# annikabrundyn/driving-dirty

Measured on AMD Instinct MI355X. Metric: 6-view scenes/sec fwd+bwd, roadmap model bs=32, higher is better.
Workload: dtype f32

## Files before the change

driving-dirty_amd/_lib.py:

```python
import ctypes as C
import os

import torch

from .build import LIB

if os.environ.get("DD_HOTPATH_LIB"):
    LIB = os.environ["DD_HOTPATH_LIB"]

_i32, _i64, _f32, _p = C.c_int32, C.c_int64, C.c_float, C.c_void_p


class ConvDesc(C.Structure):
    _fields_ = [(n, _i32) for n in ("batch", "height", "width", "cin_real", "cin_store", "cout",
                                    "ksize", "stride", "pad", "rows_per_task")]


class GConvDesc(C.Structure):
    _fields_ = [(n, _i32) for n in ("batch", "in_h", "in_w", "in_cstore", "in_coff", "cin", "out_h", "out_w",
                                    "omem_h", "omem_w", "out_cstore", "out_coff", "cout", "kh", "kw", "stride_h",
                                    "stride_w", "dil_h", "dil_w", "pad_h", "pad_w", "div_h", "div_w", "ostride_h",
                                    "ostride_w", "ooff_h", "ooff_w", "mask_pass_lo", "mask_pass_hi")]


class AdamTensor(C.Structure):
    _fields_ = [("p", _p), ("g", _p), ("m", _p), ("v", _p), ("n", _i64)]


_DP = C.POINTER(ConvDesc)
_GP = C.POINTER(GConvDesc)

SIGNATURES = {
    "dd_abi_version": (_i32, []),
    "dd_last_error": (C.c_char_p, []),
    "dd_clock_probe": (_i32, [_p, _i32, _i32, _p]),
    "dd_set_cu_budget": (_i32, [_i32]),
    "dd_set_adam_blocks_per_cu": (_i32, [_i32]),
    "dd_set_adam_spare_cus": (_i32, [_i32]),
    "dd_get_cu_budget": (_i32, []),
    "dd_stitch6": (_i32, [_p, _p, _p, _p, _i32, _i32, _i32, _i32, _p]),
    "dd_stitch6_ptrs": (_i32, [_p, _p, _i32, _i32, _i32, _p]),
    "dd_boxes_to_binary_map": (_i32, [_p, _i32, _p, _p, _i32, _p]),
    "dd_stitch6_u8": (_i32, [_p, _p, _i32, _i32, _i32, _p]),
    "dd_stitch6_u8_ptrs": (_i32, [_p, _p, _p, _i32, _i32, _i32, _i32, _p]),
    "dd_nchw_to_nhwc": (_i32, [_p, _p, _i32, _i32, _i32, _i32, _i32, _p]),
    "dd_subsample_nhwc4": (_i32, [_p, _p, _i32, _i32, _i32, _i32, _i32, _i32, _i32, _p]),
    "dd_subsample_nhwc4_u8_ptrs": (_i32, [_p, _p, _i32, _i32, _i32, _i32, _i32, _i32, _i32, _p]),
    "dd_copy_channels": (_i32, [_p, _p, _i64, _i32, _i32, _i32, _i32, _i32, _p]),
    "dd_copy_channels_window": (_i32, [_p, _p] + [_i32] * 16 + [_p]),
    "dd_deconv2x2_c32_fwd": (_i32, [_p, _p, _p, _p, _i32, _i32, _i32, _i32, _p]),
    "dd_deconv2x2_c32_fwd_slice": (_i32, [_p, _p, _p, _p, _i32, _i32, _i32, _i32, _i32, _i32, _p]),
    "dd_deconv2x2_c32_wgrad_workspace_bytes": (_i64, []),
    "dd_deconv2x2_c32_wgrad": (_i32, [_p, _p, _p, _p, _i32, _i32, _i32, _i32, _i32, _p, _i64, _p]),
    "dd_ssconv_dgrad_supported": (_i32, [_i32, _i32, _i32]),
    "dd_ssconv_dgrad": (_i32, [_p, _p, _p, _i32, _i32, _i32, _i32, _p]),
    "dd_ssconv_fwd": (_i32, [_p, _p, _p, _p, _i32, _i32, _i32, _i32, _i32, _p]),
    "dd_conv1x1_c32_c3_nchw": (_i32, [_p, _p, _p, _p, _i32, _i32, _i32, _p]),
    "dd_conv1ch_fwd": (_i32, [_p, _p, _p, _p, _i32, _i32, _i32, _i32, _p]),
    "dd_conv1ch_wgrad_workspace_bytes": (_i64, []),
    "dd_conv1ch_fwd_phase3": (_i32, [_p, _p, _p, _p, _p, _i32, _i32, _i32, _i32, _p]),
    "dd_conv1ch_wgrad_phase3": (_i32, [_p, _p, _p, _p, _i32, _i32, _i32, _p, _p]),
    "dd_phase3_scatter": (_i32, [_p, _p] + [_i32] * 8 + [_p]),
    "dd_phase3_gather": (_i32, [_p, _p] + [_i32] * 8 + [_p]),
    "dd_conv1ch_wgrad": (_i32, [_p, _p, _p, _p, _i32, _i32, _i32, _p, _p]),
    "dd_nhwc_to_nchw": (_i32, [_p, _p, _i32, _i32, _i32, _i32, _i32, _p]),
    "dd_conv_packed_floats": (_i64, [_DP, _i32]),
    "dd_conv_pack": (_i32, [_p, _p, _DP, _i32, _p]),
    "dd_conv_fwd": (_i32, [_p, _p, _p, _p, _p, _DP, _i32, _p]),
    "dd_conv_fwd_relu_bits": (_i32, [_p, _p, _p, _p, _p, _DP, _p]),
    "dd_conv_dgrad_relu_bits": (_i32, [_p, _p, _p, _p, _DP, _p]),
    "dd_conv_stats_floats": (_i64, []),
    "dd_conv_fwd_stats": (_i32, [_p, _p, _p, _p, _p, _p, _DP, _p]),
    "dd_bn2d_finalize": (_i32, [_p, _i64, _p, _p, _p, _p, _f32, _f32, _i32, _p, _p, _p, _p]),
    "dd_bn2d_stats": (_i32, [_p, _p, _i64, _p]),
    "dd_bn2d_apply_relu": (_i32, [_p, _p, _p, _i64, _p]),
    "dd_bn2d_workspace_bytes": (_i64, []),
    "dd_bn2d_bwd": (_i32, [_p, _p, _p, _p, _p, _p, _p, _p, _i64, _i32, _p, _p]),
    "dd_conv_dgrad_bn": (_i32, [_p, _p, _p, _p, _p, _DP, _p]),
    "dd_conv_wgrad_bn": (_i32, [_p, _p, _p, _p, _p, _p, _i64, _DP, _p]),
    "dd_pool4_bn_fwd": (_i32, [_p, _p, _p, _i32, _i32, _i32, _p]),
    "dd_pool4_bn_bwd": (_i32, [_p, _p, _p, _p, _i32, _i32, _i32, _p]),
    "dd_conv_dgrad": (_i32, [_p, _p, _p, _p, _DP, _p]),
    "dd_conv_wgrad_workspace_bytes": (_i64, [_DP]),
    "dd_conv_wgrad": (_i32, [_p, _p, _p, _p, _p, _i64, _DP, _p]),
    "dd_relu_bwd": (_i32, [_p, _p, _p, _i64, _p]),
    "dd_relu_sign_bits": (_i32, [_p, _p, _i64, _p]),
    "dd_relu_bwd_pad_bits": (_i32, [_p, _p, _p, _i32, _i32, _i32, _i32, _i32, _p]),
    "dd_pool4_fwd": (_i32, [_p, _p, _i32, _i32, _i32, _i32, _p]),
    "dd_pool4_relu_bwd": (_i32, [_p, _p, _p, _i32, _i32, _i32, _i32, _p]),
    "dd_pool4_relu_bwd_add": (_i32, [_p, _p, _p, _p, _i32, _i32, _i32, _i32, _p]),
    "dd_pool4_idx_elems": (_i64, [_i32, _i32, _i32, _i32]),
    "dd_pool4_fwd_idx": (_i32, [_p, _p, _p, _i32, _i32, _i32, _i32, _p]),
    "dd_pool4_idx_relu_bwd": (_i32, [_p, _p, _p, _i32, _i32, _i32, _i32, _p]),
    "dd_mlp_tail_supported": (_i32, [_i32] * 4),
    "dd_mlp_tail_fwd": (_i32, [_p] * 25 + [_i32] * 4 + [_f32] * 6 + [_i32, _p]),
    "dd_mlp_tail_bwd": (_i32, [_p] * 28 + [_i32] * 4 + [_f32] * 4 + [_i32, _p]),
    "dd_bn_relu_drop_fwd": (_i32, [_p] * 9 + [_i32, _i32, _f32, _f32, _f32, _i32, _p, _p]),
    "dd_bn_relu_drop_bwd": (_i32, [_p] * 12 + [_i32, _i32, _f32, _f32, _i32, _p]),
    "dd_loss_workspace_bytes": (_i64, [_i64]),
    "dd_bce_logits": (_i32, [_p, _p, _p, _p, _p, _i64, _f32, _p, _p]),
    "dd_bce_logits_u8": (_i32, [_p, _p, _p, _p, _p, _i64, _f32, _p, _p]),
    "dd_bce_logits_u8_ptrs": (_i32, [_p, _p, _i32, _i64, _p, _p, _p, _f32, _p, _p]),
    "dd_scale_by_device_scalar": (_i32, [_p, _p, _i64, _p]),
    "dd_sigmoid": (_i32, [_p, _p, _i64, _p]),
    "dd_sigmoid_bwd": (_i32, [_p, _p, _p, _i64, _p]),
    "dd_mse": (_i32, [_p, _p, _p, _p, _i64, _f32, _p, _p]),
    "dd_gconv_packed_floats": (_i64, [_GP]),
    "dd_gconv_pack": (_i32, [_p, _p, _GP, _i64, _i64, _i64, _i32, _i32, _i32, _p]),
    "dd_gconv_fwd": (_i32, [_p, _p, _p, _p, _p, _GP, _i32, _p]),
    "dd_gconv_wgrad_workspace_bytes": (_i64, [_GP]),
    "dd_gconv_wgrad": (_i32, [_p, _p, _p, _p, _GP, _i64, _i64, _i64, _i32, _i32, _i32, _i32, _p, _i64, _p]),
    "dd_dconv_supported": (_i32, [_GP]),
    "dd_dconv_packed_floats": (_i64, [_GP]),
    "dd_dconv_pack": (_i32, [_p, _p, _GP, _i64, _i64, _i64, _i32, _i32, _i32, _p]),
    "dd_dconv_fwd": (_i32, [_p, _p, _p, _p, _p, _GP, _i32, _p]),
    "dd_dconv_colsum_supported": (_i32, [_p, _i32, _i32]),
    "dd_dconv_colsum_workspace_bytes": (_i64, []),
    "dd_dconv_fwd_colsum": (_i32, [_p, _p, _p, _p, _p, _p, _i32, _p, _i64, _p]),
    "dd_dconv_split_supported": (_i32, [_GP]),
    "dd_dconv_split_input_bytes": (_i64, [_GP]),
    "dd_dconv_split_packed_bytes": (_i64, [_GP]),
    "dd_dconv_split_input": (_i32, [_p, _p, _GP, _p]),
    "dd_dconv_split_pack": (_i32, [_p, _p, _GP, _i64, _i64, _i64, _i32, _i32, _i32, _p]),
# ... 114 lines not shown
```

driving-dirty_amd/csrc/conv3x3.hip:

```cpp
#include <stdlib.h>

#include "dd_common.h"

namespace {

constexpr int EPI_BIAS_RELU_BITS = 5;
constexpr int EPI_RELU_BITS = 6;
constexpr int EPI_BIAS_STATS = 7;
constexpr int EPI_RELU_MASK_AFF = 8;
constexpr int EPI_RELU_BITS_W1 = 9;


template <int CIN, int S>
struct StripCfg {
  static constexpr int PXB = CIN * 4;
  static constexpr int CHUNKS = CIN / 4;
  static constexpr int NPX = 32 * S + 2;
  static constexpr int SLOTB = NPX * PXB;
  static constexpr int NCH = NPX * CHUNKS;
  static constexpr int NLOAD = (NCH + 63) / 64;
  static constexpr int SPILLB = (NLOAD * 64 - NCH) * 16;
  static constexpr int WAVEB = 3 * SLOTB + SPILLB;
  static constexpr int KGROUPS = (CIN == 32) ? 36 : 5;
  static constexpr int WFLOATS = KGROUPS * 64 * 4;
// ... 1789 lines not shown
}

__global__ __launch_bounds__(256) void relu_sign_bits_kernel(const float* __restrict__ x, unsigned* __restrict__ bits, long npix) {
  const int lane = threadIdx.x & 63;
  const long wave = ((long)blockIdx.x * blockDim.x + threadIdx.x) >> 6, nwaves = ((long)gridDim.x * blockDim.x) >> 6;
  for (long p0 = wave * 64; p0 < npix; p0 += nwaves * 64) {
    unsigned word = 0;
#pragma unroll 8
    for (int i = 0; i < 32; ++i) {
      const long p = p0 + 2 * i + (lane >> 5);
      const float v = p < npix ? x[p * 32 + (lane & 31)] : 0.f;
      const unsigned long long m = __ballot(v > 0.f);
      if (lane == 2 * i) word = (unsigned)m;
      if (lane == 2 * i + 1) word = (unsigned)(m >> 32);
    }
    if (p0 + lane < npix) bits[p0 + lane] = word;
  }
}

__global__ __launch_bounds__(256) void relu_bwd_pad_bits_kernel(const float* __restrict__ dy, const unsigned* __restrict__ bits_pad,
                                                                f32x4* __restrict__ out_pad, int B, int H, int W, int dy_cstore, int dy_coff) {
  const long total = (long)B * (H + 2) * (W + 2) * 8;
  for (long i = (long)blockIdx.x * blockDim.x + threadIdx.x; i < total; i += (long)gridDim.x * blockDim.x) {
    const int q = (int)(i & 7);
    const long pp = i >> 3;
    const int xx = (int)(pp % (W + 2)), yy = (int)((pp / (W + 2)) % (H + 2));
    const long b = pp / ((long)(W + 2) * (H + 2));
    f32x4 o = {0.f, 0.f, 0.f, 0.f};
    if (xx >= 1 && xx <= W && yy >= 1 && yy <= H) {
      const f32x4 g = *(const f32x4*)(dy + ((b * H + (yy - 1)) * W + (xx - 1)) * dy_cstore + dy_coff + 4 * q);
      const unsigned m = bits_pad[pp] >> (4 * q);
      o.x = (m & 1u) ? g.x : 0.f;
      o.y = (m & 2u) ? g.y : 0.f;
      o.z = (m & 4u) ? g.z : 0.f;
      o.w = (m & 8u) ? g.w : 0.f;
    }
    __builtin_nontemporal_store(o, out_pad + i);
  }
}

__global__ void relu_bwd_kernel(const f32x4* __restrict__ dy, const f32x4* __restrict__ y, f32x4* __restrict__ out,
                                long n4) {
  for (long i = (long)blockIdx.x * blockDim.x + threadIdx.x; i < n4; i += (long)gridDim.x * blockDim.x) {
    const f32x4 g = dy[i], v = y[i];
    f32x4 o;
    o.x = v.x > 0.f ? g.x : 0.f;
    o.y = v.y > 0.f ? g.y : 0.f;
    o.z = v.z > 0.f ? g.z : 0.f;
    o.w = v.w > 0.f ? g.w : 0.f;
    out[i] = o;
  }
}

int check_desc(const dd_conv_desc* d) {
  DD_REQUIRE(d != nullptr, DD_ERR_BAD_ARG, "conv: NULL descriptor");
  DD_REQUIRE(d->batch > 0 && d->height > 0 && d->width > 0, DD_ERR_BAD_ARG, "conv: non-positive size");
  DD_REQUIRE(d->ksize == 3 && d->pad == 1, DD_ERR_UNSUPPORTED, "conv: only k3 p1 is implemented (got k%d p%d)", d->ksize, d->pad);
  DD_REQUIRE(d->stride == 1 || d->stride == 2, DD_ERR_UNSUPPORTED, "conv: stride %d", d->stride);
  DD_REQUIRE(d->cout == 32, DD_ERR_UNSUPPORTED, "conv: Cout %d (only 32)", d->cout);
  DD_REQUIRE((d->cin_real == 32 && d->cin_store == 32) || (d->cin_real == 3 && d->cin_store == 4), DD_ERR_UNSUPPORTED,
             "conv: Cin %d stored as %d (supported: 32/32, 3/4)", d->cin_real, d->cin_store);
  DD_REQUIRE(!(d->cin_real == 3 && d->stride == 2), DD_ERR_UNSUPPORTED, "conv: Cin 3 with stride 2");
  DD_REQUIRE((long)d->width * 128 < (1L << 31), DD_ERR_UNSUPPORTED, "conv: row too long for a 32-bit buffer descriptor");
  return 0;
}

int resident_grid(const dd_conv_desc* d, long row_tiles, int wpb, int per_cu) {
  long blocks = (long)dd_cu_budget_internal() * per_cu;
  if (d->rows_per_task > 0) blocks = min(blocks, max(1L, row_tiles / d->rows_per_task / wpb));
  return (int)max(1L, min(blocks, (row_tiles + wpb - 1) / wpb));
}

template <int CIN, int S, int EPI, int WPB, bool AFF = false>
int launch_fwd(const float* x, const float* wp, const float* bias, const float* msk, float* y, const dd_conv_desc* d,
               hipStream_t st, unsigned* bits_out = nullptr, const float* aff = nullptr, float* stats = nullptr) {
  using C = StripCfg<CIN, S>;
  const int Ho = dd_conv_out(d->height, S), Wo = dd_conv_out(d->width, S);
  const int nstrips = (Wo + 31) / 32;
  const size_t lds = C::WFLOATS * 4 + (size_t)WPB * C::WAVEB;
  const int per_cu = (int)max((size_t)1, min((size_t)2, (size_t)(160 * 1024) / lds));
  const int grid = resident_grid(d, (long)d->batch * nstrips * Ho, WPB, per_cu);
  auto k = conv_strip_fwd<CIN, S, EPI, WPB, AFF>;
  if (int rc = dd_allow_lds((const void*)k, lds)) return rc;
  hipLaunchKernelGGL(k, dim3(grid), dim3(WPB * 64), lds, st, x, wp, bias, msk, y, bits_out, d->batch, d->height, d->width,
                     Ho, Wo, nstrips, aff, stats);
  DD_LAUNCH_CHECK("conv_strip_fwd");
  return 0;
}

template <int MASK>
int launch_s2_dgrad(const float* dy, const float* packed_dgrad, const float* relu_src, float* dx, const dd_conv_desc* d, hipStream_t st,
                    const float* aff) {
  using C = StripCfg<32, 1>;
  constexpr int WPB = 8;
  const int H = d->height, W = d->width, Ho = dd_conv_out(H, 2), Wo = dd_conv_out(W, 2);
  const int ns = (W + 1) / 2, nr = (H + 1) / 2;
  const int nstrips = (ns + 31) / 32;
  const size_t lds = C::WFLOATS * 4 + (size_t)WPB * C::WAVEB;
  const int grid = resident_grid(d, (long)d->batch * nstrips * nr, WPB, 1);
  auto k = conv_s2_dgrad<WPB, MASK>;
  if (int rc = dd_allow_lds((const void*)k, lds)) return rc;
  hipLaunchKernelGGL(k, dim3(grid), dim3(WPB * 64), lds, st, dy, packed_dgrad, relu_src, dx, d->batch, H, W, Ho, Wo, nstrips, aff);
  DD_LAUNCH_CHECK("conv_s2_dgrad");
  return 0;
}

template <int EPI>
int launch_wino2(const float* x, const float* up, const float* bias, const unsigned* bits_in, float* y, unsigned* bits_out,
                 const dd_conv_desc* d, hipStream_t st, const float* x4 = nullptr, float* w1part = nullptr, int* nw_out = nullptr) {
  using C = StripCfg<32, 1>;
  using C4 = StripCfg<4, 1>;
  constexpr int WPB = 4;
  const int nstrips = (d->width + 31) / 32;
  static const bool ring_env = getenv("DD_WINO2_RING") != nullptr;
  static const bool ring_w1 = getenv("DD_WINO2_RING_W1") != nullptr;
  const bool ring = ring_env || (EPI == EPI_RELU_BITS_W1 && ring_w1);
  DD_REQUIRE((long)d->height * d->width * 128 < (1L << 30), DD_ERR_UNSUPPORTED, "conv_wino2: image of %d x %d pixels: the kernel addresses an image with 30-bit offsets",
             d->height, d->width);
  const size_t lds = (size_t)WINO2_UFLOATS * 4 + (ring ? (size_t)WPB * (4 * C::SLOTB + C::SPILLB) : 0) +
                     (EPI == EPI_RELU_BITS_W1 ? (size_t)WPB * (4 * C4::SLOTB + C4::SPILLB) + 128 : 0);
  const int grid = resident_grid(d, (long)d->batch * nstrips * ((d->height + 1) / 2), WPB, 1);
  if (nw_out) *nw_out = grid * WPB;
  if (int rc = dd_allow_lds(ring ? (const void*)conv_wino2_fwd<EPI, WPB> : (const void*)conv_wino2r_fwd<EPI, WPB>, lds)) return rc;
  constexpr int pf_rows = 1;
  auto kring = conv_wino2_fwd<EPI, WPB>;
  auto kreg = conv_wino2r_fwd<EPI, WPB>;
  if (ring) hipLaunchKernelGGL(kring, dim3(grid), dim3(WPB * 64), lds, st, x, up, bias, bits_in, y, bits_out, d->batch, d->height, d->width, nstrips, x4, w1part);
  else hipLaunchKernelGGL(kreg, dim3(grid), dim3(WPB * 64), lds, st, x, up, bias, bits_in, y, bits_out, d->batch, d->height, d->width, nstrips, x4, w1part, pf_rows);
  DD_LAUNCH_CHECK("conv_wino2_fwd");
  return 0;
}

template <int EPI>
int launch_wino(const float* x, const float* up, const float* bias, const unsigned* bits_in, float* y, unsigned* bits_out,
                const dd_conv_desc* d, hipStream_t st) {
  using C = StripCfg<32, 1>;
  constexpr int WPB = 8;
  const int nstrips = (d->width + 31) / 32;
  const size_t lds = (size_t)WINO_UFLOATS * 4 + (size_t)WPB * C::WAVEB;
// ... 8 lines not shown
}

extern "C" {

int64_t dd_conv_packed_floats(const dd_conv_desc* d, int32_t kind) {
  if (check_desc(d)) return -1;
  if (kind != 0 && d->cin_real != 32) return -1;
  return d->cin_real == 32 ? 36 * 64 * 4 : 5 * 64 * 4;
}

int dd_conv_pack(const float* w_oihw, float* packed, const dd_conv_desc* d, int32_t kind, void* stream) {
  if (int rc = check_desc(d)) return rc;
  DD_REQUIRE(w_oihw && packed, DD_ERR_BAD_ARG, "conv_pack: NULL pointer");
  DD_REQUIRE(kind >= 0 && kind <= 2, DD_ERR_BAD_ARG, "conv_pack: kind %d", kind);
  DD_REQUIRE(kind == 0 || d->cin_real == 32, DD_ERR_UNSUPPORTED, "conv_pack: dgrad packing needs Cin 32");
  const int n = d->cin_real == 32 ? 36 * 64 * 4 : 5 * 64 * 4;
  hipLaunchKernelGGL(conv_pack_kernel, dim3((n + 255) / 256), dim3(256), 0, (hipStream_t)stream, w_oihw, packed,
                     d->cin_real, kind);
  DD_LAUNCH_CHECK("conv_pack");
  return 0;
}

int dd_conv_fwd(const float* x, const float* packed_fwd, const float* bias, const float* mask, float* y,
                const dd_conv_desc* d, int32_t epilogue, void* stream) {
  if (int rc = check_desc(d)) return rc;
  DD_REQUIRE(x && packed_fwd && y, DD_ERR_BAD_ARG, "conv_fwd: NULL pointer");
  DD_REQUIRE(epilogue != DD_EPI_RELU_MASK || mask, DD_ERR_BAD_ARG, "conv_fwd: RELU_MASK epilogue needs a mask");
  DD_REQUIRE((epilogue != DD_EPI_BIAS && epilogue != DD_EPI_BIAS_RELU) || bias, DD_ERR_BAD_ARG, "conv_fwd: bias epilogue needs a bias");
  hipStream_t st = (hipStream_t)stream;
#define DD_DISPATCH(CIN, S, WPB)                                                                                    \
  switch (epilogue) {                                                                                               \
    case DD_EPI_NONE: return launch_fwd<CIN, S, DD_EPI_NONE, WPB>(x, packed_fwd, bias, mask, y, d, st);             \
    case DD_EPI_BIAS: return launch_fwd<CIN, S, DD_EPI_BIAS, WPB>(x, packed_fwd, bias, mask, y, d, st);             \
    case DD_EPI_BIAS_RELU: return launch_fwd<CIN, S, DD_EPI_BIAS_RELU, WPB>(x, packed_fwd, bias, mask, y, d, st);   \
    case DD_EPI_RELU_MASK: return launch_fwd<CIN, S, DD_EPI_RELU_MASK, WPB>(x, packed_fwd, bias, mask, y, d, st);   \
    default: return dd_fail(DD_ERR_BAD_ARG, "conv_fwd: epilogue %d", epilogue);                                     \
  }
  if (d->cin_store == 4) { DD_DISPATCH(4, 1, 8) }
  if (d->stride == 1) { DD_DISPATCH(32, 1, 8) }
  DD_DISPATCH(32, 2, 4)
#undef DD_DISPATCH
}

int dd_conv_fwd_relu_bits(const float* x, const float* packed_fwd, const float* bias, float* y, uint32_t* relu_bits,
                          const dd_conv_desc* d, void* stream) {
  if (int rc = check_desc(d)) return rc;
  DD_REQUIRE(x && packed_fwd && bias && y && relu_bits, DD_ERR_BAD_ARG, "conv_fwd_relu_bits: NULL pointer");
  hipStream_t st = (hipStream_t)stream;
  if (d->cin_store == 4) return launch_fwd<4, 1, EPI_BIAS_RELU_BITS, 8>(x, packed_fwd, bias, nullptr, y, d, st, relu_bits);
  if (d->stride == 1) return launch_fwd<32, 1, EPI_BIAS_RELU_BITS, 8>(x, packed_fwd, bias, nullptr, y, d, st, relu_bits);
  return launch_fwd<32, 2, EPI_BIAS_RELU_BITS, 4>(x, packed_fwd, bias, nullptr, y, d, st, relu_bits);
}

static int conv_dgrad_impl(const float* dy, const float* packed_dgrad, const float* relu_src, int mask_mode, float* dx,
                           const dd_conv_desc* d, void* stream, const float* aff = nullptr);

int dd_conv_dgrad(const float* dy, const float* packed_dgrad, const float* relu_src, float* dx, const dd_conv_desc* d,
                  void* stream) {
  return conv_dgrad_impl(dy, packed_dgrad, relu_src, relu_src ? 1 : 0, dx, d, stream);
}

int dd_conv_dgrad_relu_bits(const float* dy, const float* packed_dgrad, const uint32_t* relu_bits, float* dx,
                            const dd_conv_desc* d, void* stream) {
  DD_REQUIRE(relu_bits, DD_ERR_BAD_ARG, "conv_dgrad_relu_bits: NULL mask");
  return conv_dgrad_impl(dy, packed_dgrad, (const float*)relu_bits, 2, dx, d, stream);
}

int dd_conv_dgrad_bn(const float* dy, const float* packed_dgrad, const float* pre_bn, const float* affine, float* dx,
                     const dd_conv_desc* d, void* stream) {
  DD_REQUIRE(pre_bn && affine, DD_ERR_BAD_ARG, "conv_dgrad_bn: NULL mask / affine");
  return conv_dgrad_impl(dy, packed_dgrad, pre_bn, 3, dx, d, stream, affine);
}

static int conv_dgrad_impl(const float* dy, const float* packed_dgrad, const float* relu_src, int mask_mode, float* dx,
                           const dd_conv_desc* d, void* stream, const float* aff) {
  if (int rc = check_desc(d)) return rc;
  DD_REQUIRE(dy && packed_dgrad && dx, DD_ERR_BAD_ARG, "conv_dgrad: NULL pointer");
  DD_REQUIRE(d->cin_real == 32, DD_ERR_UNSUPPORTED, "conv_dgrad: Cin %d (the first layer has no data gradient)", d->cin_real);
  hipStream_t st = (hipStream_t)stream;
  if (d->stride == 1) {
    if (mask_mode == 3) return launch_fwd<32, 1, EPI_RELU_MASK_AFF, 8>(dy, packed_dgrad, nullptr, relu_src, dx, d, st, nullptr, aff);
    if (mask_mode == 2) return launch_fwd<32, 1, EPI_RELU_BITS, 8>(dy, packed_dgrad, nullptr, relu_src, dx, d, st);
    return mask_mode ? launch_fwd<32, 1, DD_EPI_RELU_MASK, 8>(dy, packed_dgrad, nullptr, relu_src, dx, d, st)
                     : launch_fwd<32, 1, DD_EPI_NONE, 8>(dy, packed_dgrad, nullptr, nullptr, dx, d, st);
  }
  switch (mask_mode) {
    case 3: return launch_s2_dgrad<3>(dy, packed_dgrad, relu_src, dx, d, st, aff);
    case 2: return launch_s2_dgrad<2>(dy, packed_dgrad, relu_src, dx, d, st, aff);
    case 1: return launch_s2_dgrad<1>(dy, packed_dgrad, relu_src, dx, d, st, aff);
    default: return launch_s2_dgrad<0>(dy, packed_dgrad, relu_src, dx, d, st, aff);
  }
}

int64_t dd_conv_wgrad_workspace_bytes(const dd_conv_desc* d) {
  if (check_desc(d)) return -1;
  const int nt = d->cin_real == 32 ? 9 : 1;
  const int64_t waves = 4 * (int64_t)DD_NUM_CU * 2;
  return waves * ((int64_t)nt * 1024 + 64) * 4;
}

static int conv_wgrad_impl(const float* x, const float* aff, const float* dy, float* dw_oihw, float* dbias, void* workspace,
                           int64_t workspace_bytes, const dd_conv_desc* d, void* stream);

int dd_conv_wgrad(const float* x, const float* dy, float* dw_oihw, float* dbias, void* workspace,
                  int64_t workspace_bytes, const dd_conv_desc* d, void* stream) {
  return conv_wgrad_impl(x, nullptr, dy, dw_oihw, dbias, workspace, workspace_bytes, d, stream);
// ... 277 lines not shown
```

driving-dirty_amd/ops.py:

```python
import ctypes as C
import os

import torch

from . import _lib
from . import ddp as _ddp
from ._lib import ConvDesc, check

EPI_NONE, EPI_BIAS, EPI_BIAS_RELU, EPI_RELU_MASK = 0, 1, 2, 3
PACK_FWD, PACK_DGRAD_S1, PACK_DGRAD_S2 = 0, 1, 2


def _stream():
    return C.c_void_p(torch.cuda.current_stream().cuda_stream)


def _p(t):
    if t is None:
        return None
    ptr = t.data_ptr()
    if _ddp.PARAM_WAITS:
        wait = _ddp.PARAM_WAITS.pop(ptr, None)
        if wait is not None:
            wait()
# ... 351 lines not shown
    return out


def nhwc_to_nchw(x, c):
    b, h, w, cs = x.shape
    _dev(x, "x")
    out = torch.empty((b, c, h, w), device=x.device, dtype=torch.float32)
    check(_lib.lib().dd_nhwc_to_nchw(_p(x), _p(out), b, c, h, w, cs, _stream()), "dd_nhwc_to_nchw")
    return out


class ToNHWC(torch.autograd.Function):

    @staticmethod
    def forward(ctx, x, c_store):
        ctx.c = x.shape[1]
        return nchw_to_nhwc(x.contiguous(), c_store)

    @staticmethod
    def backward(ctx, g):
        return nhwc_to_nchw(g.contiguous(), ctx.c), None


def conv_pack(weight, desc, kind):
    _dev(weight, "weight", (32, desc.cin_real, 3, 3))
    n = _lib.lib().dd_conv_packed_floats(C.byref(desc), kind)
    if n <= 0:
        raise _lib.HotpathError(f"conv_pack: {_lib.lib().dd_last_error().decode()}")
    packed = torch.empty(n, device=weight.device, dtype=torch.float32)
    check(_lib.lib().dd_conv_pack(_p(weight), _p(packed), C.byref(desc), kind, _stream()), "dd_conv_pack")
    return packed


def conv_fwd(x, packed, bias, desc, epilogue=EPI_BIAS_RELU, mask=None):
    ho, wo = conv_out(desc.height, desc.stride), conv_out(desc.width, desc.stride)
    _dev(x, "x", (desc.batch, desc.height, desc.width, desc.cin_store))
    if bias is not None:
        _dev(bias, "bias", (32,))
    if mask is not None:
        _dev(mask, "mask", (desc.batch, ho, wo, 32))
    y = torch.empty((desc.batch, ho, wo, 32), device=x.device, dtype=torch.float32)
    check(_lib.lib().dd_conv_fwd(_p(x), _p(packed), _p(bias), _p(mask), _p(y), C.byref(desc), epilogue, _stream()), "dd_conv_fwd")
    return y


def conv_fwd_bits(x, packed, bias, desc):
    ho, wo = conv_out(desc.height, desc.stride), conv_out(desc.width, desc.stride)
    _dev(x, "x", (desc.batch, desc.height, desc.width, desc.cin_store))
    _dev(bias, "bias", (32,))
    y = torch.empty((desc.batch, ho, wo, 32), device=x.device, dtype=torch.float32)
    bits = torch.empty((desc.batch, ho, wo), device=x.device, dtype=torch.int32)
    check(_lib.lib().dd_conv_fwd_relu_bits(_p(x), _p(packed), _p(bias), _p(y), _p(bits), C.byref(desc), _stream()), "dd_conv_fwd_relu_bits")
    return y, bits


WINOGRAD = True
WINOGRAD_2D = True


def conv_wino_pack(weight, desc, kind):
    _dev(weight, "weight", (32, 32, 3, 3))
    n = _lib.lib().dd_conv_wino_packed_floats(C.byref(desc))
    if n <= 0:
        raise _lib.HotpathError(f"conv_wino_pack: {_lib.lib().dd_last_error().decode()}")
    packed = torch.empty(n, device=weight.device, dtype=torch.float32)
    check(_lib.lib().dd_conv_wino_pack(_p(weight), _p(packed), C.byref(desc), kind, _stream()), "dd_conv_wino_pack")
    return packed


def conv_wino_fwd_bits(x, packed, bias, desc):
    _dev(x, "x", (desc.batch, desc.height, desc.width, 32))
    _dev(bias, "bias", (32,))
    y = torch.empty((desc.batch, desc.height, desc.width, 32), device=x.device, dtype=torch.float32)
    bits = torch.empty((desc.batch, desc.height, desc.width), device=x.device, dtype=torch.int32)
    check(_lib.lib().dd_conv_wino_fwd_relu_bits(_p(x), _p(packed), _p(bias), _p(y), _p(bits), C.byref(desc), _stream()),
          "dd_conv_wino_fwd_relu_bits")
    return y, bits


def conv_wino_dgrad_bits(dy, packed, bits, desc):
    _dev(dy, "dy", (desc.batch, desc.height, desc.width, 32))
    if not (bits.is_cuda and bits.dtype == torch.int32 and bits.is_contiguous() and tuple(bits.shape) == (desc.batch, desc.height, desc.width)):
        raise _lib.HotpathError("conv_wino_dgrad_bits: relu_bits must be a contiguous int32 [B,H,W] device tensor")
    dx = torch.empty((desc.batch, desc.height, desc.width, 32), device=dy.device, dtype=torch.float32)
    check(_lib.lib().dd_conv_wino_dgrad_relu_bits(_p(dy), _p(packed), _p(bits), _p(dx), C.byref(desc), _stream()),
          "dd_conv_wino_dgrad_relu_bits")
    return dx


def conv_wino2_pack(weight, desc, kind):
    _dev(weight, "weight", (32, 32, 3, 3))
    n = _lib.lib().dd_conv_wino2_packed_floats(C.byref(desc))
    if n <= 0:
        raise _lib.HotpathError(f"conv_wino2_pack: {_lib.lib().dd_last_error().decode()}")
    packed = torch.empty(n, device=weight.device, dtype=torch.float32)
    check(_lib.lib().dd_conv_wino2_pack(_p(weight), _p(packed), C.byref(desc), kind, _stream()), "dd_conv_wino2_pack")
    return packed


def conv_wino2_fwd_bits(x, packed, bias, desc):
    _dev(x, "x", (desc.batch, desc.height, desc.width, 32))
    _dev(bias, "bias", (32,))
    y = torch.empty((desc.batch, desc.height, desc.width, 32), device=x.device, dtype=torch.float32)
    bits = torch.empty((desc.batch, desc.height, desc.width), device=x.device, dtype=torch.int32)
    check(_lib.lib().dd_conv_wino2_fwd_relu_bits(_p(x), _p(packed), _p(bias), _p(y), _p(bits), C.byref(desc), _stream()),
          "dd_conv_wino2_fwd_relu_bits")
# ... 211 lines not shown

_PACK_STREAMS = {}


def _pack_stream(device):
    key = torch.device(device).index
    if key not in _PACK_STREAMS:
        _PACK_STREAMS[key] = torch.cuda.Stream(device=device)
    return _PACK_STREAMS[key]


class EncoderConvStack(torch.autograd.Function):

    @staticmethod
    def forward(ctx, x4, w1, b1, w2, b2, w3, b3, pool, rows_per_task):
        b, h, w, _ = x4.shape
        d1 = conv_desc(b, h, w, 3, 1, rows_per_task)
        d2 = conv_desc(b, h, w, 32, 1, rows_per_task)
        d3 = conv_desc(b, h, w, 32, 2, rows_per_task)
        need = ctx.needs_input_grad
        p1 = conv_pack(w1, d1, PACK_FWD)
        main = torch.cuda.current_stream()
        side = _pack_stream(x4.device)
        side.wait_event(main.record_event())
        with torch.cuda.stream(side):
            if WINOGRAD and WINOGRAD_2D:
                p2 = conv_wino2_pack(w2, d2, 0)
            elif WINOGRAD:
                p2 = conv_wino_pack(w2, d2, 0)
            else:
                p2 = conv_pack(w2, d2, PACK_FWD)
            p3 = conv_pack(w3, d3, PACK_FWD)
            p2d = p3d = torch.empty(0, device=x4.device)
            if need[1] or need[2] or need[3] or need[4]:
                p3d = conv_pack(w3, d3, PACK_DGRAD_S2)
            if need[1] or need[2]:
                if WINOGRAD and WINOGRAD_2D:
                    p2d = conv_wino2_pack(w2, d2, 1)
                elif WINOGRAD:
                    p2d = conv_wino_pack(w2, d2, 1)
                else:
                    p2d = conv_pack(w2, d2, PACK_DGRAD_S1)
            for t in (p2, p3, p2d, p3d):
                t.record_stream(main)
            packed_ready = side.record_event()
        a1, s1 = conv_fwd_bits(x4, p1, b1, d1)
        main.wait_event(packed_ready)
        if WINOGRAD and WINOGRAD_2D:
            a2, s2 = conv_wino2_fwd_bits(a1, p2, b2, d2)
        elif WINOGRAD:
            a2, s2 = conv_wino_fwd_bits(a1, p2, b2, d2)
        else:
            a2, s2 = conv_fwd_bits(a1, p2, b2, d2)
        a3 = conv_fwd(a2, p3, b3, d3)
        if TRACE is not None:
            TRACE.update(a1=a1, a2=a2, a3=a3)
        ctx.wino = (bool(WINOGRAD), bool(WINOGRAD and WINOGRAD_2D))
        ctx.pool = int(pool)
        ctx.rows_per_task = rows_per_task
        ctx.a3_shape = tuple(a3.shape)
        if ctx.pool == 1 and pool4_has_idx(*a3.shape[1:]):
            pooled, codes = pool4_fwd_idx(a3)
            ctx.save_for_backward(x4, a1, a2, codes, p2d, p3d, s1, s2)
            ctx.codes = True
            return pooled
        ctx.codes = False
        ctx.save_for_backward(x4, a1, a2, a3, p2d, p3d, s1, s2)
        if ctx.pool == 2:
            return a3, pool4_fwd(a3)
        if ctx.pool:
            return pool4_fwd(a3)
        return a3

    @staticmethod
    def backward(ctx, grad, grad_pooled=None):
        x4, a1, a2, a3, p2d, p3d, s1, s2 = ctx.saved_tensors
        wino, wino2 = ctx.wino
        b, h, w, _ = x4.shape
        rpt = ctx.rows_per_task
        d1, d2, d3 = conv_desc(b, h, w, 3, 1, rpt), conv_desc(b, h, w, 32, 1, rpt), conv_desc(b, h, w, 32, 2, rpt)
        if ctx.pool == 2:
            if grad is not None and grad_pooled is not None and a3.shape[3] == 32 and (a3.shape[1] * a3.shape[2]) % 4 == 0:
                g3 = pool4_relu_bwd_add(grad_pooled.contiguous(), a3, grad.contiguous())
            else:
                parts = []
                if grad is not None:
                    parts.append(relu_bwd(grad.contiguous(), a3))
                if grad_pooled is not None:
                    parts.append(pool4_relu_bwd(grad_pooled.contiguous(), a3))
                g3 = parts[0] if len(parts) == 1 else add(parts[0], parts[1])
        else:
            grad = grad.contiguous()
            if ctx.codes:
                g3 = pool4_idx_relu_bwd(grad, a3, ctx.a3_shape)
            else:
                g3 = pool4_relu_bwd(grad, a3) if ctx.pool else relu_bwd(grad, a3)
        need = ctx.needs_input_grad
        dw3, db3 = conv_wgrad(a2, g3, d3) if (need[5] or need[6]) else (None, None)
        dw2 = db2 = dw1 = db1 = None
        if need[1] or need[2] or need[3] or need[4]:
            g2 = conv_dgrad_bits(g3, p3d, s2, d3)
            del g3
            for hook in MFMA_PHASE_HOOKS:
                hook()
            reduced = None

            def c2_weight_gradient():
                nonlocal dw2, db2, reduced
                if need[3] or need[4]:
                    if wino2:
                        dw2, db2, reduced = conv_wino2_wgrad(a1, g2, d2, finish_stream=_pack_stream(g2.device))
                    elif wino:
# ... 425 lines not shown
```

include/dd_hotpath.h:

```cpp
#ifndef DD_HOTPATH_H
#define DD_HOTPATH_H

#include <stdint.h>

#ifdef __cplusplus
extern "C" {
#endif

#define DD_ABI_VERSION 4

enum {
  DD_OK = 0,
  DD_ERR_UNSUPPORTED = 1,
  DD_ERR_BAD_ARG = 2,
  DD_ERR_LAUNCH = 3,
  DD_ERR_WORKSPACE = 4
};

enum {
  DD_EPI_NONE = 0,
  DD_EPI_BIAS = 1,
  DD_EPI_BIAS_RELU = 2,
  DD_EPI_RELU_MASK = 3
};

typedef struct dd_conv_desc {
  int32_t batch, height, width;
  int32_t cin_real, cin_store, cout;
  int32_t ksize, stride, pad;
  int32_t rows_per_task;
} dd_conv_desc;

int dd_abi_version(void);
const char* dd_last_error(void);

int dd_clock_probe(uint64_t* samples, int32_t nsamples, int32_t spin, void* stream);

int dd_set_cu_budget(int32_t compute_units);
int dd_get_cu_budget(void);
int dd_set_adam_blocks_per_cu(int32_t blocks);
int dd_set_adam_spare_cus(int32_t compute_units);

int dd_stitch6(const float* views, float* wide_nhwc4, float* wide_nchw, float* target,
               int32_t batch, int32_t height, int32_t width, int32_t mask_slot, void* stream);

int dd_stitch6_ptrs(const float* const* sample_ptrs, float* wide_nhwc4, int32_t batch, int32_t height, int32_t width,
                    void* stream);

int dd_boxes_to_binary_map(const void* boxes, int32_t boxes_dtype, const int32_t* sample_offsets, float* maps,
                           int32_t batch, void* stream);

int dd_stitch6_u8(const unsigned char* frames, float* wide_nhwc4, int32_t batch, int32_t height, int32_t width,
                  void* stream);
int dd_stitch6_u8_ptrs(const unsigned char* const* sample_ptrs, float* wide_nhwc4, float* target, int32_t batch, int32_t height,
                       int32_t width, int32_t mask_slot, void* stream);

int dd_nchw_to_nhwc(const float* src, float* dst, int32_t batch, int32_t c, int32_t h, int32_t w,
                    int32_t c_store, void* stream);
int dd_nhwc_to_nchw(const float* src, float* dst, int32_t batch, int32_t c, int32_t h, int32_t w,
                    int32_t c_store, void* stream);

int64_t dd_conv_packed_floats(const dd_conv_desc* d, int32_t kind);
int dd_conv_pack(const float* w_oihw, float* packed, const dd_conv_desc* d, int32_t kind, void* stream);

int dd_conv_fwd(const float* x, const float* packed_fwd, const float* bias, const float* mask,
                float* y, const dd_conv_desc* d, int32_t epilogue, void* stream);

int dd_conv_dgrad(const float* dy, const float* packed_dgrad, const float* relu_src, float* dx,
                  const dd_conv_desc* d, void* stream);

int dd_conv_fwd_relu_bits(const float* x, const float* packed_fwd, const float* bias, float* y, uint32_t* relu_bits,
                          const dd_conv_desc* d, void* stream);
int dd_conv_dgrad_relu_bits(const float* dy, const float* packed_dgrad, const uint32_t* relu_bits, float* dx,
                            const dd_conv_desc* d, void* stream);

int64_t dd_conv_stats_floats(void);
int dd_conv_fwd_stats(const float* x, const float* packed_fwd, const float* bias, const float* in_affine, float* u,
                      float* stats, const dd_conv_desc* d, void* stream);
int dd_bn2d_finalize(const float* stats, int64_t count, const float* gamma, const float* beta, float* running_mean,
                     float* running_var, float momentum, float eps, int32_t training, float* affine, float* save_mean,
                     float* save_invstd, void* stream);
int dd_bn2d_stats(const float* u, float* stats, int64_t npix, void* stream);
int dd_bn2d_apply_relu(const float* u, const float* affine, float* y, int64_t npix, void* stream);
int64_t dd_bn2d_workspace_bytes(void);
int dd_bn2d_bwd(const float* g, const float* u, const float* gamma, const float* save_mean, const float* save_invstd,
                float* du, float* dgamma, float* dbeta, int64_t npix, int32_t training, void* workspace, void* stream);
int dd_conv_dgrad_bn(const float* dy, const float* packed_dgrad, const float* pre_bn, const float* affine, float* dx,
                     const dd_conv_desc* d, void* stream);
int dd_conv_wgrad_bn(const float* pre_bn, const float* affine, const float* dy, float* dw_oihw, float* dbias, void* workspace,
                     int64_t workspace_bytes, const dd_conv_desc* d, void* stream);
int dd_pool4_bn_fwd(const float* u, const float* affine, float* pooled, int32_t batch, int32_t h, int32_t w, void* stream);
int dd_pool4_bn_bwd(const float* dpooled, const float* u, const float* affine, float* dfeat, int32_t batch, int32_t h, int32_t w,
                    void* stream);

int64_t dd_conv_wgrad_workspace_bytes(const dd_conv_desc* d);
int dd_conv_wgrad(const float* x, const float* dy, float* dw_oihw, float* dbias, void* workspace,
                  int64_t workspace_bytes, const dd_conv_desc* d, void* stream);

int dd_relu_bwd(const float* dy, const float* y, float* out, int64_t n, void* stream);

int dd_relu_sign_bits(const float* x, uint32_t* bits, int64_t npix, void* stream);
int dd_relu_bwd_pad_bits(const float* dy, const uint32_t* bits_pad, float* out_pad, int32_t batch, int32_t h, int32_t w, int32_t dy_cstore,
                         int32_t dy_coff, void* stream);

int dd_pool4_fwd(const float* feat, float* pooled, int32_t batch, int32_t h, int32_t w, int32_t c,
                 void* stream);
int dd_pool4_relu_bwd(const float* dpooled, const float* feat, float* dfeat, int32_t batch, int32_t h,
                      int32_t w, int32_t c, void* stream);
int dd_pool4_relu_bwd_add(const float* dpooled, const float* feat, const float* gfeat, float* dfeat, int32_t batch, int32_t h, int32_t w,
                          int32_t c, void* stream);
int64_t dd_pool4_idx_elems(int32_t batch, int32_t h, int32_t w, int32_t c);
int dd_pool4_fwd_idx(const float* feat, float* pooled, uint16_t* idx, int32_t batch, int32_t h, int32_t w, int32_t c,
                     void* stream);
int dd_pool4_idx_relu_bwd(const float* dpooled, const uint16_t* idx, float* dfeat, int32_t batch, int32_t h, int32_t w,
                          int32_t c, void* stream);

int dd_bn_relu_drop_fwd(const float* x, const float* gamma, const float* beta, float* running_mean,
                        float* running_var, const float* keep, float* y, float* save_mean,
                        float* save_invstd, int32_t rows, int32_t feat, float eps, float momentum,
                        float scale, int32_t training, int64_t* num_batches_tracked, void* stream);
int dd_bn_relu_drop_bwd(const float* dy, const float* x, const float* y, const float* gamma,
                        const float* keep, const float* save_mean, const float* save_invstd,
                        const float* running_mean, const float* running_var, float* dx, float* dgamma, float* dbeta, int32_t rows,
                        int32_t feat, float eps, float scale, int32_t training, void* stream);

int dd_mlp_tail_supported(int32_t m, int32_t h1, int32_t h2, int32_t l);
int dd_mlp_tail_fwd(const float* lin1, const float* gamma1, const float* beta1, float* running_mean1, float* running_var1,
// ... 269 lines not shown
```

Before: 4394.

## Fuse stride-2 conv3 forward with 4-wide max-pool and index codes

Adds a dedicated kernel that computes the third 32->32 stride-2 conv with bias+ReLU and directly reduces each group of four consecutive pixels into pooled maxima plus packed argmax/positive codes. The full-resolution a3 activation is never written to or reread from global memory. Pool windows that straddle row boundaries go through a small edge workspace and a second fix-up kernel. The fused path is enabled by default for pool mode 1 and falls back to the old path when unsupported. It adds a custom LDS ring layout and edge-case handling complexity.

```diff
diff --git a/driving-dirty_amd/_lib.py b/driving-dirty_amd/_lib.py
--- a/driving-dirty_amd/_lib.py
+++ b/driving-dirty_amd/_lib.py
@@ -69,6 +69,8 @@
     "dd_conv_fwd": (_i32, [_p, _p, _p, _p, _p, _DP, _i32, _p]),
     "dd_conv_fwd_relu_bits": (_i32, [_p, _p, _p, _p, _p, _DP, _p]),
     "dd_conv_dgrad_relu_bits": (_i32, [_p, _p, _p, _p, _DP, _p]),
+    "dd_conv_fwd_pool4_workspace_bytes": (_i64, [_DP]),
+    "dd_conv_fwd_pool4": (_i32, [_p, _p, _p, _p, _p, _p, _i64, _DP, _p]),
     "dd_conv_stats_floats": (_i64, []),
     "dd_conv_fwd_stats": (_i32, [_p, _p, _p, _p, _p, _p, _DP, _p]),
     "dd_bn2d_finalize": (_i32, [_p, _i64, _p, _p, _p, _p, _f32, _f32, _i32, _p, _p, _p, _p]),
diff --git a/driving-dirty_amd/csrc/conv3x3.hip b/driving-dirty_amd/csrc/conv3x3.hip
--- a/driving-dirty_amd/csrc/conv3x3.hip
+++ b/driving-dirty_amd/csrc/conv3x3.hip
@@ -1865,6 +1865,187 @@
   }
 }
 
+struct PoolStripCfg {
+  static constexpr int NPX = 72;
+  static constexpr int SLOTB = NPX * 128;
+  static constexpr int NLOAD = NPX * 8 / 64;
+  static constexpr int WAVEB = 3 * SLOTB;
+};
+
+__device__ __forceinline__ void pool_load_row(const float* __restrict__ img, int H, int W, int iy, int gxb, int nch, int lane,
+                                              f32x4 (&r)[PoolStripCfg::NLOAD]) {
+  const bool rowok = (iy >= 0) && (iy < H);
+  const __amdgpu_buffer_rsrc_t rs = dd_rsrc(img + (long)(rowok ? iy : 0) * W * 32, rowok ? W * 128 : 0);
+#pragma unroll
+  for (int i = 0; i < PoolStripCfg::NLOAD; ++i) {
+    const int c = lane + 64 * i;
+    const int q = c >> 3, ch = c & 7;
+    const int off = (c < nch) ? ((gxb + q) * 128 + ch * 16) : -16;
+    r[i] = dd_bload4<DD_AUX_NT>(rs, off);
+  }
+}
+
+__device__ __forceinline__ void pool_store_row(char* slot, int lane, const f32x4 (&r)[PoolStripCfg::NLOAD]) {
+#pragma unroll
+  for (int i = 0; i < PoolStripCfg::NLOAD; ++i) {
+    const int c = lane + 64 * i;
+    const int q = c >> 3, ch = c & 7;
+    *(f32x4*)(slot + q * 128 + ((ch ^ swz<32>(q)) << 4)) = r[i];
+  }
+}
+
+__device__ __forceinline__ unsigned pool_window(float v0, float v1, float v2, float v3, float& m) {
+  m = v0;
+  unsigned am = 0;
+  if (v1 > m) { m = v1; am = 1; }
+  if (v2 > m) { m = v2; am = 2; }
+  if (v3 > m) { m = v3; am = 3; }
+  return am | (m > 0.f ? 4u : 0u);
+}
+
+template <int WPB>
+__global__ __launch_bounds__(WPB * 64) void conv_s2_pool_fwd(const float* __restrict__ x, const float* __restrict__ wp,
+                                                             const float* __restrict__ bias, float* __restrict__ pooled,
+                                                             unsigned* __restrict__ codes, float* __restrict__ edge, int B, int H,
+                                                             int W, int Ho, int Wo, int nstrips, int shmax) {
+  using C = StripCfg<32, 2>;
+  using P = PoolStripCfg;
+  extern __shared__ __attribute__((aligned(16))) char smem[];
+  const int tid = threadIdx.x;
+  const int lane = tid & 63;
+  const int wave = __builtin_amdgcn_readfirstlane(tid >> 6);
+  {
+    f32x4* wl4 = (f32x4*)smem;
+    const f32x4* wg4 = (const f32x4*)wp;
+    for (int i = tid; i < C::WFLOATS / 4; i += WPB * 64) wl4[i] = wg4[i];
+  }
+  __syncthreads();
+  char* ring = smem + C::WFLOATS * 4 + wave * P::WAVEB;
+  const char* wl = smem;
+  const int h = lane >> 5, n = lane & 31;
+  const float bv = bias[n];
+  const int quads = Ho * Wo / 4;
+  const int nch = (66 + 2 * shmax) * 8;
+  const __amdgpu_buffer_rsrc_t es = dd_rsrc(edge, B * Ho * 512);
+
+  long idx, end;
+  dd_range((long)B * nstrips * Ho, blockIdx.x * WPB + wave, gridDim.x * WPB, idx, end);
+  while (idx < end) {
+    const long col = idx / Ho;
+    const int y0 = (int)(idx - col * Ho);
+    const int y1 = (int)min((long)Ho, y0 + (end - idx));
+    idx += y1 - y0;
+    const int b = (int)(col / nstrips), x0 = (int)(col % nstrips) * 32;
+    const float* xb = x + (long)b * H * W * 32;
+    const int gxb = 2 * x0 - 1 - 2 * shmax;
+    const __amdgpu_buffer_rsrc_t ps = dd_rsrc(pooled + (long)b * 32 * quads, quads * 128);
+    const __amdgpu_buffer_rsrc_t cs = dd_rsrc(codes + (long)b * 4 * quads, quads * 16);
+
+#pragma unroll
+    for (int d = 0; d < 3; ++d) {
+      f32x4 t[P::NLOAD];
+      const int iy = 2 * y0 - 1 + d;
+      pool_load_row(xb, H, W, iy, gxb, nch, lane, t);
+      pool_store_row(ring + ((iy + 1) % 3) * P::SLOTB, lane, t);
+    }
+
+    for (int yy = y0; yy < y1; ++yy) {
+      f32x4 pre[2][P::NLOAD];
+#pragma unroll
+      for (int s = 0; s < 2; ++s) pool_load_row(xb, H, W, 2 * yy + 2 + s, gxb, nch, lane, pre[s]);
+      __builtin_amdgcn_sched_barrier(0);
+
+      const int sh = (int)(((long)yy * Wo) & 3);
+      const int qoff = 2 * (shmax - sh);
+      f32x16 acc;
+#pragma unroll
+      for (int r = 0; r < 16; ++r) acc[r] = 0.f;
+#pragma unroll
+      for (int dy = 0; dy < 3; ++dy) {
+        const char* rowb = ring + ((2 * yy + dy) % 3) * P::SLOTB;
+#pragma unroll
+        for (int dx = 0; dx < 3; ++dx) {
+          const int q = 2 * n + dx + qoff;
+          const char* pa = rowb + q * 128;
+          const int sw = swz<32>(q);
+#pragma unroll
+          for (int j = 0; j < 4; ++j) {
+            const f32x4 a = *(const f32x4*)(pa + (((2 * j + h) ^ sw) << 4));
+            const f32x4 w = *(const f32x4*)(wl + (((dy * 3 + dx) * 4 + j) * 64 + lane) * 16);
+            acc = DD_MFMA(a.x, w.x, acc);
+            acc = DD_MFMA(a.y, w.y, acc);
+            acc = DD_MFMA(a.z, w.z, acc);
+            acc = DD_MFMA(a.w, w.w, acc);
+          }
+        }
+      }
+
+#pragma unroll
+      for (int s = 0; s < 2; ++s) pool_store_row(ring + ((2 * yy + 3 + s) % 3) * P::SLOTB, lane, pre[s]);
+
+      const int xs = x0 - sh;
+      const int wq0 = (int)(((long)yy * Wo + xs) >> 2);
+      float v[16];
+#pragma unroll
+      for (int r = 0; r < 16; ++r) v[r] = fmaxf(acc[r] + bv, 0.f);
+      unsigned word = 0;
+#pragma unroll
+      for (int g = 0; g < 4; ++g) {
+        const int wi = 2 * g + h, xf = xs + 4 * wi;
+        const bool whole = xf >= 0 && xf + 3 < Wo;
+        float m;
+        unsigned c = pool_window(v[4 * g], v[4 * g + 1], v[4 * g + 2], v[4 * g + 3], m) << (4 * (n & 7));
+        dd_bstore1(ps, whole ? (n * quads + wq0 + wi) * 4 : -16, m);
+        c |= __shfl_xor(c, 1);
+        c |= __shfl_xor(c, 2);
+        c |= __shfl_xor(c, 4);
+        if ((n & 7) == g) word = c;
+      }
+      {
+        const int g = n & 7, wi = 2 * g + h, xf = xs + 4 * wi;
+        const bool whole = g < 4 && xf >= 0 && xf + 3 < Wo;
+        __builtin_amdgcn_raw_buffer_store_b32(word, cs, whole ? ((wq0 + wi) * 4 + (n >> 3)) * 4 : -16, 0, 0);
+      }
+      const int shn = (yy + 1 < Ho) ? (int)(((long)(yy + 1) * Wo) & 3) : 0;
+      const bool head = x0 == 0 && sh > 0;
+      const bool tail = shn > 0 && Wo - shn >= xs && Wo - shn < xs + 32;
+      if (head || tail) {
+#pragma unroll
+        for (int g = 0; g < 4; ++g) {
+          const int wi = 2 * g + h, xf = xs + 4 * wi;
+          const bool ish = head && wi == 0, ist = tail && xf == Wo - shn;
+          const int erow = b * Ho + (ish ? yy : yy + 1);
+#pragma unroll
+          for (int k = 0; k < 4; ++k) {
+            const bool ok = ish ? (k >= sh) : (ist && k < shn);
+            dd_bstore1(es, ok ? ((erow * 4 + k) * 32 + n) * 4 : -16, v[4 * g + k]);
+          }
+        }
+      }
+    }
+  }
+}
+
+__global__ __launch_bounds__(256) void conv_s2_pool_edge(const float* __restrict__ edge, float* __restrict__ pooled,
+                                                         unsigned* __restrict__ codes, int B, int Ho, int Wo) {
+  const int i = blockIdx.x * 256 + threadIdx.x;
+  if (i >= B * Ho * 4) return;
+  const int c8 = i & 3, yy = (i >> 2) % Ho, b = (i >> 2) / Ho;
+  const int sh = (int)(((long)yy * Wo) & 3);
+  if (sh == 0) return;
+  const long quads = (long)Ho * Wo / 4;
+  const long wq = ((long)yy * Wo - sh) >> 2;
+  const float* e = edge + ((long)(b * Ho + yy) * 4) * 32 + 8 * c8;
+  unsigned word = 0;
+#pragma unroll
+  for (int j = 0; j < 8; ++j) {
+    float m;
+    word |= pool_window(e[j], e[32 + j], e[64 + j], e[96 + j], m) << (4 * j);
+    pooled[((long)b * 32 + 8 * c8 + j) * quads + wq] = m;
+  }
+  codes[((long)b * quads + wq) * 4 + c8] = word;
+}
+
 int check_desc(const dd_conv_desc* d) {
   DD_REQUIRE(d != nullptr, DD_ERR_BAD_ARG, "conv: NULL descriptor");
   DD_REQUIRE(d->batch > 0 && d->height > 0 && d->width > 0, DD_ERR_BAD_ARG, "conv: non-positive size");
@@ -1898,6 +2079,38 @@
   hipLaunchKernelGGL(k, dim3(grid), dim3(WPB * 64), lds, st, x, wp, bias, msk, y, bits_out, d->batch, d->height, d->width,
                      Ho, Wo, nstrips, aff, stats);
   DD_LAUNCH_CHECK("conv_strip_fwd");
+  return 0;
+}
+
+int check_pool_desc(const dd_conv_desc* d) {
+  if (int rc = check_desc(d)) return rc;
+  DD_REQUIRE(d->cin_real == 32 && d->stride == 2, DD_ERR_UNSUPPORTED, "conv_fwd_pool4: the 32 -> 32 stride-2 layer only (Cin %d, stride %d)",
+             d->cin_real, d->stride);
+  const long Ho = dd_conv_out(d->height, 2), Wo = dd_conv_out(d->width, 2);
+  DD_REQUIRE((Ho * Wo) % 4 == 0 && Wo >= 4, DD_ERR_UNSUPPORTED, "conv_fwd_pool4: needs Ho*Wo %% 4 == 0 and Wo >= 4 (got %ld x %ld)", Ho, Wo);
+  DD_REQUIRE(Ho * Wo * 32 < (1L << 31) && d->batch * Ho * 512 < (1L << 31), DD_ERR_UNSUPPORTED,
+             "conv_fwd_pool4: %d images of %ld x %ld pixels: the kernel addresses a pooled image and the edge buffer with 31-bit offsets",
+             d->batch, Ho, Wo);
+  return 0;
+}
+
+int launch_pool_fwd(const float* x, const float* wp, const float* bias, float* pooled, unsigned* codes, float* edge,
+                    const dd_conv_desc* d, hipStream_t st) {
+  constexpr int WPB = 4;
+  const int Ho = dd_conv_out(d->height, 2), Wo = dd_conv_out(d->width, 2);
+  const int shmax = (Wo % 4 == 0 || Ho == 1) ? 0 : (Wo % 2 == 0 ? 2 : 3);
+  const int nstrips = (Wo + shmax + 31) / 32;
+  const size_t lds = StripCfg<32, 2>::WFLOATS * 4 + (size_t)WPB * PoolStripCfg::WAVEB;
+  const int grid = resident_grid(d, (long)d->batch * nstrips * Ho, WPB, 1);
+  auto k = conv_s2_pool_fwd<WPB>;
+  if (int rc = dd_allow_lds((const void*)k, lds)) return rc;
+  hipLaunchKernelGGL(k, dim3(grid), dim3(WPB * 64), lds, st, x, wp, bias, pooled, codes, edge, d->batch, d->height, d->width, Ho, Wo,
+                     nstrips, shmax);
+  DD_LAUNCH_CHECK("conv_s2_pool_fwd");
+  if (shmax > 0) {
+    hipLaunchKernelGGL(conv_s2_pool_edge, dim3((d->batch * Ho * 4 + 255) / 256), dim3(256), 0, st, edge, pooled, codes, d->batch, Ho, Wo);
+    DD_LAUNCH_CHECK("conv_s2_pool_edge");
+  }
   return 0;
 }
 
@@ -2012,6 +2225,21 @@
   return launch_fwd<32, 2, EPI_BIAS_RELU_BITS, 4>(x, packed_fwd, bias, nullptr, y, d, st, relu_bits);
 }
 
+int64_t dd_conv_fwd_pool4_workspace_bytes(const dd_conv_desc* d) {
+  if (check_pool_desc(d)) return -1;
+  return (int64_t)d->batch * dd_conv_out(d->height, 2) * 512;
+}
+
+int dd_conv_fwd_pool4(const float* x, const float* packed_fwd, const float* bias, float* pooled, uint16_t* idx, void* workspace,
+                      int64_t workspace_bytes, const dd_conv_desc* d, void* stream) {
+  if (int rc = check_pool_desc(d)) return rc;
+  DD_REQUIRE(x && packed_fwd && bias && pooled && idx && workspace, DD_ERR_BAD_ARG, "conv_fwd_pool4: NULL pointer");
+  DD_REQUIRE(workspace_bytes >= dd_conv_fwd_pool4_workspace_bytes(d), DD_ERR_WORKSPACE, "conv_fwd_pool4: workspace %ld < %ld bytes",
+             (long)workspace_bytes, (long)dd_conv_fwd_pool4_workspace_bytes(d));
+  DD_REQUIRE((((uintptr_t)idx | (uintptr_t)workspace) & 3) == 0, DD_ERR_BAD_ARG, "conv_fwd_pool4: idx and workspace must be 4-byte aligned");
+  return launch_pool_fwd(x, packed_fwd, bias, pooled, (unsigned*)idx, (float*)workspace, d, (hipStream_t)stream);
+}
+
 static int conv_dgrad_impl(const float* dy, const float* packed_dgrad, const float* relu_src, int mask_mode, float* dx,
                            const dd_conv_desc* d, void* stream, const float* aff = nullptr);
 
diff --git a/driving-dirty_amd/ops.py b/driving-dirty_amd/ops.py
--- a/driving-dirty_amd/ops.py
+++ b/driving-dirty_amd/ops.py
@@ -427,6 +427,24 @@
     bits = torch.empty((desc.batch, ho, wo), device=x.device, dtype=torch.int32)
     check(_lib.lib().dd_conv_fwd_relu_bits(_p(x), _p(packed), _p(bias), _p(y), _p(bits), C.byref(desc), _stream()), "dd_conv_fwd_relu_bits")
     return y, bits
+
+
+FUSE_C3_POOL_FWD = os.environ.get("DD_C3_POOL_FWD", "1") != "0"
+
+
+def conv_fwd_pool4(x, packed, bias, desc):
+    _dev(x, "x", (desc.batch, desc.height, desc.width, desc.cin_store))
+    _dev(bias, "bias", (32,))
+    nbytes = _lib.lib().dd_conv_fwd_pool4_workspace_bytes(C.byref(desc))
+    if nbytes < 0:
+        return None
+    ho, wo = conv_out(desc.height, desc.stride), conv_out(desc.width, desc.stride)
+    pooled = torch.empty((desc.batch, 32 * ho * wo // 4), device=x.device, dtype=torch.float32)
+    idx = torch.empty((desc.batch * (ho * wo // 4) * 8,), device=x.device, dtype=torch.int16)
+    ws = torch.empty(nbytes, device=x.device, dtype=torch.uint8)
+    check(_lib.lib().dd_conv_fwd_pool4(_p(x), _p(packed), _p(bias), _p(pooled), _p(idx), _p(ws), nbytes, C.byref(desc), _stream()),
+          "dd_conv_fwd_pool4")
+    return pooled, idx
 
 
 WINOGRAD = True
@@ -744,12 +762,20 @@
             a2, s2 = conv_wino_fwd_bits(a1, p2, b2, d2)
         else:
             a2, s2 = conv_fwd_bits(a1, p2, b2, d2)
+        ctx.wino = (bool(WINOGRAD), bool(WINOGRAD and WINOGRAD_2D))
+        ctx.pool = int(pool)
+        ctx.rows_per_task = rows_per_task
+        if ctx.pool == 1 and FUSE_C3_POOL_FWD and TRACE is None:
+            fused = conv_fwd_pool4(a2, p3, b3, d3)
+            if fused is not None:
+                pooled, codes = fused
+                ctx.a3_shape = (b, conv_out(h, 2), conv_out(w, 2), 32)
+                ctx.save_for_backward(x4, a1, a2, codes, p2d, p3d, s1, s2)
+                ctx.codes = True
+                return pooled
         a3 = conv_fwd(a2, p3, b3, d3)
         if TRACE is not None:
             TRACE.update(a1=a1, a2=a2, a3=a3)
-        ctx.wino = (bool(WINOGRAD), bool(WINOGRAD and WINOGRAD_2D))
-        ctx.pool = int(pool)
-        ctx.rows_per_task = rows_per_task
         ctx.a3_shape = tuple(a3.shape)
         if ctx.pool == 1 and pool4_has_idx(*a3.shape[1:]):
             pooled, codes = pool4_fwd_idx(a3)
diff --git a/include/dd_hotpath.h b/include/dd_hotpath.h
--- a/include/dd_hotpath.h
+++ b/include/dd_hotpath.h
@@ -73,6 +73,10 @@
                           const dd_conv_desc* d, void* stream);
 int dd_conv_dgrad_relu_bits(const float* dy, const float* packed_dgrad, const uint32_t* relu_bits, float* dx,
                             const dd_conv_desc* d, void* stream);
+
+int64_t dd_conv_fwd_pool4_workspace_bytes(const dd_conv_desc* d);
+int dd_conv_fwd_pool4(const float* x, const float* packed_fwd, const float* bias, float* pooled, uint16_t* idx, void* workspace,
+                      int64_t workspace_bytes, const dd_conv_desc* d, void* stream);
 
 int64_t dd_conv_stats_floats(void);
 int dd_conv_fwd_stats(const float* x, const float* packed_fwd, const float* bias, const float* in_affine, float* u,
```

Result: no change. 4378 (median of 2 runs) (-0.4%).
